# rsasaki0109/lidarslam_ros2

Measured on AMD Instinct MI355X. Metric: scan registrations/sec (30k-pt scan vs 10-frame submap), higher is better.
Workload: dtype f32; 1 GPU; cfg2: single NDT align(), 30000-pt VLP-32 scan (vg 0.2) vs 10-frame submap (vg 0.1), ndt_resolution 5.0, DIRECT7, max_iterations 30, transformation_epsilon 0; 1018 different scans (stream of 64); target_points=661519, voxels_valid=643, derivative_passes_last_scan=242, parallelism=1 registration stream per GPU x1, collective=none (one rank)

## Files before the change

lidarslam_ros2_amd/csrc/ndt.hip:

```cpp
#include "ndt.hpp"

#include <cmath>
#include <cstdlib>
#include <type_traits>

#include "grid_device.hpp"
#include "ndt_point.hpp"
#include "sort.hpp"

namespace lsr {

namespace {

__host__ __device__ inline void angle_tables(const double* p, bool with_hessian, int d1_sign, float* jang, float* hang) {
  double cx, cy, cz, sx, sy, sz;
  if (fabs(p[3]) < 10e-5) { cx = 1.0; sx = 0.0; } else { cx = cos(p[3]); sx = sin(p[3]); }
  if (fabs(p[4]) < 10e-5) { cy = 1.0; sy = 0.0; } else { cy = cos(p[4]); sy = sin(p[4]); }
  if (fabs(p[5]) < 10e-5) { cz = 1.0; sz = 0.0; } else { cz = cos(p[5]); sz = sin(p[5]); }
  jang[0] = (float)(-sx * sz + cx * sy * cz); jang[1] = (float)(-sx * cz - cx * sy * sz); jang[2] = (float)(-cx * cy);
  jang[3] = (float)(cx * sz + sx * sy * cz);  jang[4] = (float)(cx * cz - sx * sy * sz);  jang[5] = (float)(-sx * cy);
  jang[6] = (float)(-sy * cz);                jang[7] = (float)(sy * sz);                 jang[8] = (float)(cy);
  jang[9] = (float)(sx * cy * cz);            jang[10] = (float)(-sx * cy * sz);          jang[11] = (float)(sx * sy);
  jang[12] = (float)(-cx * cy * cz);          jang[13] = (float)(cx * cy * sz);           jang[14] = (float)(-cx * sy);
  jang[15] = (float)(-cy * sz);               jang[16] = (float)(-cy * cz);               jang[17] = 0.f;
// ... 413 lines not shown
  const double psi_t = phi_t - phi_0 - mu * d_phi_0 * a_t;
  const double d_psi_t = d_phi_t - mu * d_phi_0;
  if (phase == PH_MT_TRIAL || phase == PH_MT_LAST) {
    if (open_interval && (psi_t <= 0 && d_psi_t >= 0)) {
      open_interval = 0;
      I.f_l = I.f_l + phi_0 - mu * d_phi_0 * I.a_l;
      I.g_l = I.g_l + mu * d_phi_0;
      I.f_u = I.f_u + phi_0 - mu * d_phi_0 * I.a_u;
      I.g_u = I.g_u + mu * d_phi_0;
    }
    if (open_interval)
      interval_converged = mt_update_interval(I, a_t, psi_t, d_psi_t) ? 1 : 0;
    else
      interval_converged = mt_update_interval(I, a_t, phi_t, d_phi_t) ? 1 : 0;
    step_iterations++;
  }
  int next = CTL_DONE;
  if (!interval_converged && step_iterations < max_step_iterations && !(psi_t <= 0 && d_phi_t <= -nu * d_phi_0)) {
    if (open_interval)
      a_t = mt_trial_value(I.a_l, I.f_l, I.g_l, I.a_u, I.f_u, I.g_u, a_t, psi_t, d_psi_t);
    else
      a_t = mt_trial_value(I.a_l, I.f_l, I.g_l, I.a_u, I.f_u, I.g_u, a_t, phi_t, d_phi_t);
    a_t = fmax(fmin(a_t, step_max), step_min);
#pragma unroll
    for (int i = 0; i < 6; i++) S->x_t[i] = p[i] + dir[i] * a_t;
    S->a_t = a_t;
    const bool last = step_iterations + 1 >= max_step_iterations;
    S->want_hessian = last ? NDT_PASS_FUSED : NDT_PASS_GRAD;
    S->phase = last ? PH_MT_LAST : PH_MT_TRIAL;
    S->pad1 = 1;
  } else if (phase == PH_MT_LAST) {
    next = CTL_NEWTON_END;
  } else if (step_iterations) {
    S->want_hessian = 1;
    S->phase = PH_MT_HESS;
  } else {
    next = CTL_NEWTON_END;
  }
  S->n_evals = n_evals;
  S->n_passes = n_passes;
  S->last_pairs = sv[7];
  S->score = score;
#pragma unroll
  for (int i = 0; i < 6; i++) S->g[i] = sv[1 + i];
  S->open_interval = open_interval;
  S->interval_converged = interval_converged;
  S->step_iterations = step_iterations;
  S->a_l = I.a_l; S->f_l = I.f_l; S->g_l = I.g_l; S->a_u = I.a_u; S->f_u = I.f_u; S->g_u = I.g_u;
  return next;
}

__device__ __forceinline__ int ndt_newton_end(LdsState* S) {
  const int nr_iterations = S->nr_iterations, max_iter = S->max_iter;
  const double a_t = S->a_t, eps = S->eps;
  double p[6], dir[6];
#pragma unroll
  for (int i = 0; i < 6; i++) { p[i] = S->p[i]; dir[i] = S->dir[i]; }
  const double score = S->score;
  const int n_points = S->n_points;
  int converged = S->converged;
  if (nr_iterations > max_iter || (nr_iterations && (fabs(a_t) < eps))) converged = 1;
#pragma unroll
  for (int i = 0; i < 6; i++) S->p[i] = p[i] + dir[i] * a_t;
  S->nr_iterations = nr_iterations + 1;
  S->converged = converged;
  if (converged) {
    S->trans_probability = score / (double)n_points;
    S->done = 1;
    return CTL_DONE;
  }
  return CTL_NEWTON_BEGIN;
}

__device__ __forceinline__ int ndt_newton_begin(LdsState* S, const LdsDouble* delta_lds) {
  const double mu = 1.e-4;
  double delta[6], g[6], p[6];
#pragma unroll
  for (int i = 0; i < 6; i++) { delta[i] = delta_lds[i]; g[i] = S->g[i]; p[i] = S->p[i]; }
  const double score = S->score, step_max = S->step_max, step_min = S->step_min;
  const int n_points = S->n_points;
  double nrm = 0;
#pragma unroll
  for (int i = 0; i < 6; i++) nrm += delta[i] * delta[i];
  nrm = sqrt(nrm);
  if (nrm == 0 || nrm != nrm) {
    S->converged = (nrm == nrm) ? 1 : 0;
    S->trans_probability = score / (double)n_points;
    S->done = 1;
    return CTL_DONE;
  }
  double dir[6];
#pragma unroll
  for (int i = 0; i < 6; i++) dir[i] = delta[i] / nrm;
  const double phi_0 = -score;
  double dot = 0;
#pragma unroll
  for (int i = 0; i < 6; i++) dot += g[i] * dir[i];
  double d_phi_0 = -dot;
  S->phi_0 = phi_0;
  if (d_phi_0 >= 0) {
    if (d_phi_0 == 0) {
      S->d_phi_0 = d_phi_0;
      S->a_t = 0;
#pragma unroll
      for (int i = 0; i < 6; i++) S->dir[i] = dir[i];
      return CTL_NEWTON_END;
    }
    d_phi_0 = -d_phi_0;
#pragma unroll
    for (int i = 0; i < 6; i++) dir[i] = -dir[i];
  }
  const double a_t = fmax(fmin(nrm, step_max), step_min);
  S->d_phi_0 = d_phi_0;
  S->a_l = 0; S->a_u = 0;
  S->f_l = 0; S->f_u = 0;
  S->g_l = d_phi_0 - mu * d_phi_0;
  S->g_u = d_phi_0 - mu * d_phi_0;
  S->interval_converged = (step_max - step_min) < 0 ? 1 : 0;
  S->open_interval = 1;
  S->step_iterations = 0;
  S->a_t = a_t;
#pragma unroll
  for (int i = 0; i < 6; i++) { S->dir[i] = dir[i]; S->x_t[i] = p[i] + dir[i] * a_t; }
  S->want_hessian = 1;
  S->phase = PH_MT_FIRST;
  S->pad1 = 3;
  return CTL_DONE;
}

__device__ __forceinline__ void ndt_controller_wave0(LdsState* S, const LdsDouble* sums) {
  const bool lead = (threadIdx.x == 0);
  int next = 0;
  if (lead) next = ndt_controller_mt(S, sums);
  next = __builtin_amdgcn_readfirstlane(next);
  LdsDouble* scratch = const_cast<LdsDouble*>(sums);
  for (int guard = 0; guard < 8 && next != CTL_DONE; guard++) {
    if (next == CTL_NEWTON_END) {
      if (lead) next = ndt_newton_end(S);
    } else {
      asm volatile("s_waitcnt lgkmcnt(0)" ::: "memory");
      __builtin_amdgcn_wave_barrier();
      solve6_wave(sums + 8, S->g, scratch);
      asm volatile("s_waitcnt lgkmcnt(0)" ::: "memory");
      __builtin_amdgcn_wave_barrier();
      if (lead) next = ndt_newton_begin(S, scratch);
    }
    next = __builtin_amdgcn_readfirstlane(next);
  }
  if (lead && next != CTL_DONE) {
    S->trans_probability = S->score / (double)S->n_points;
    S->done = 1;
  }
}

#ifdef LSR_TIMING
__device__ long long* g_lsr_timing = nullptr;
#define LSR_STAMP(k)                                                                   \
  if (threadIdx.x == 0 && g_lsr_timing && blockIdx.y == 0) {                            \
    g_lsr_timing[blockIdx.x * 32 + 2 * (k)] = (long long)wall_clock64();                \
    g_lsr_timing[blockIdx.x * 32 + 2 * (k) + 1] = (long long)clock64();                 \
  }
#define LSR_STAMP_T(k, t)                                                              \
  if ((int)threadIdx.x == (t) && g_lsr_timing && blockIdx.y == 0) {                       \
    g_lsr_timing[blockIdx.x * 32 + 2 * (k)] = (long long)wall_clock64();                \
  }
#ifdef LSR_TIMING_SPAN
#define LSR_SPAN_BEGIN(seq)                                                                                   \
  if (threadIdx.x == 0 && g_lsr_timing && blockIdx.y == 0)                                                     \
    atomicMin((unsigned long long*)&g_lsr_timing[(512 + ((seq) & 255)) * 32 + 0], (unsigned long long)wall_clock64());
#define LSR_SPAN_END(seq)                                                                                     \
  if (threadIdx.x == 0 && g_lsr_timing && blockIdx.y == 0)                                                     \
    atomicMax((unsigned long long*)&g_lsr_timing[(512 + ((seq) & 255)) * 32 + 1], (unsigned long long)wall_clock64());
#else
#define LSR_SPAN_BEGIN(seq)
#define LSR_SPAN_END(seq)
#endif
#define LSR_CTL_BEGIN(L)                                                              \
  long long _ctl_t0 = 0; int _ctl_ph = 0;                                              \
  if (threadIdx.x == 0 && g_lsr_timing && blockIdx.x == 0 && blockIdx.y == 0) { _ctl_t0 = (long long)wall_clock64(); _ctl_ph = (L)->phase; }
#define LSR_CTL_END(col)                                                              \
  if (threadIdx.x == 0 && g_lsr_timing && blockIdx.x == 0 && blockIdx.y == 0) {          \
    const long long _t = (long long)wall_clock64();                                     \
    atomicAdd((unsigned long long*)&g_lsr_timing[(800 + _ctl_ph) * 32 + (col)], (unsigned long long)(_t - _ctl_t0)); \
    if ((col) == 0) atomicAdd((unsigned long long*)&g_lsr_timing[(800 + _ctl_ph) * 32 + 1], 1ull);                     \
    _ctl_t0 = _t;                                                                       \
  }
#define LSR_PASS_BEGIN()                                                               \
  long long _p_t0 = 0, _p_c0 = 0, _p_t1 = 0, _p_t7 = 0, _p_t2 = 0;                         \
  const bool _p_on = (threadIdx.x == 0 && g_lsr_timing && blockIdx.x == 0 && blockIdx.y == 0); \
  if (_p_on) { _p_t0 = (long long)wall_clock64(); _p_c0 = (long long)clock64(); }
#define LSR_PASS_MARK(var) if (_p_on) { var = (long long)wall_clock64(); }
#define LSR_PASS_END(hess)                                                             \
  if (_p_on) {                                                                          \
    const long long _t3 = (long long)wall_clock64(), _c3 = (long long)clock64();         \
    unsigned long long* _r = (unsigned long long*)&g_lsr_timing[(810 + ((hess) ? 1 : 0)) * 32]; \
    atomicAdd(&_r[0], 1ull); atomicAdd(&_r[1], (unsigned long long)(_p_t1 - _p_t0)); atomicAdd(&_r[2], (unsigned long long)(_p_t2 - _p_t7)); \
    atomicAdd(&_r[3], (unsigned long long)(_t3 - _p_t2)); atomicAdd(&_r[4], (unsigned long long)(_c3 - _p_c0)); atomicAdd(&_r[5], (unsigned long long)(_t3 - _p_t0)); \
  }
#else
#define LSR_STAMP(k)
#define LSR_STAMP_T(k, t)
#define LSR_SPAN_BEGIN(seq)
#define LSR_SPAN_END(seq)
#define LSR_CTL_BEGIN(L)
#define LSR_CTL_END(col)
#define LSR_PASS_BEGIN()
#define LSR_PASS_MARK(var)
#define LSR_PASS_END(hess)
#endif

__device__ __forceinline__ int uniform_i(int v) { return __builtin_amdgcn_readfirstlane(v); }
__device__ __forceinline__ float uniform_f(float v) { return __int_as_float(__builtin_amdgcn_readfirstlane(__float_as_int(v))); }
__device__ __forceinline__ double uniform_d(double v) {
  const int lo = __builtin_amdgcn_readfirstlane(__double2loint(v)), hi = __builtin_amdgcn_readfirstlane(__double2hiint(v));
  return __hiloint2double(hi, lo);
}

template <int CTRL>
__device__ __forceinline__ double dpp_quad_xor(double v) {
  int lo = __double2loint(v), hi = __double2hiint(v);
  lo = __builtin_amdgcn_update_dpp(0, lo, CTRL, 0xF, 0xF, true);
  hi = __builtin_amdgcn_update_dpp(0, hi, CTRL, 0xF, 0xF, true);
  return __hiloint2double(hi, lo);
}

template <int NOFF>
struct Offsets;
template <>
struct Offsets<1> {
  static __device__ __forceinline__ void get(int o, int& dx, int& dy, int& dz) { dx = dy = dz = 0; }
};
template <>
struct Offsets<7> {
  static __device__ __forceinline__ void get(int o, int& dx, int& dy, int& dz) {
    dx = (o == 1) - (o == 2);
    dy = (o == 3) - (o == 4);
    dz = (o == 5) - (o == 6);
  }
};
template <>
struct Offsets<27> {
  static __device__ __forceinline__ void get(int o, int& dx, int& dy, int& dz) {
    dx = o / 9 - 1;
    dy = (o / 3) % 3 - 1;
    dz = o % 3 - 1;
  }
};

namespace canon {
constexpr int TILE_PITCH = 68;
constexpr int TILE_ROWS = 16;
constexpr int TILE_FLOATS = TILE_ROWS * TILE_PITCH;

__device__ __forceinline__ double quantum(const int k) { return __hiloint2double((1023 + 62 - 31 * (k + 1)) << 20, 0); }
__device__ __forceinline__ double iquantum(const int k) { return __hiloint2double((1023 - 62 + 31 * (k + 1)) << 20, 0); }

__device__ __forceinline__ int piece(const double t, const int k, bool* poison) {
  *poison = !(fabs(t) < 4611686018427387904.0);
  if (*poison) return 0;
  double r = t;
  if (k > 0) r = t - trunc(t * iquantum(k - 1)) * quantum(k - 1);
  return (int)(r * iquantum(k));
}

__device__ __forceinline__ double reduce_grad(const float* p) {
  typedef float f4 __attribute__((ext_vector_type(4)));
  const f4 a = *reinterpret_cast<const f4*>(p), b = *reinterpret_cast<const f4*>(p + 4);
  double t = (double)a.x;
  t += (double)a.y; t += (double)a.z; t += (double)a.w;
  t += (double)b.x; t += (double)b.y; t += (double)b.z; t += (double)b.w;
  t += dpp_quad_xor<0xB1>(t);
  t += dpp_quad_xor<0x4E>(t);
  t += dpp_quad_xor<0x141>(t);
  return t;
}
__device__ __forceinline__ double reduce_hess(const float* p) {
  typedef float f4 __attribute__((ext_vector_type(4)));
  const f4 a = *reinterpret_cast<const f4*>(p), b = *reinterpret_cast<const f4*>(p + 4), c = *reinterpret_cast<const f4*>(p + 8),
           d = *reinterpret_cast<const f4*>(p + 12);
  double t = (double)a.x;
  t += (double)a.y; t += (double)a.z; t += (double)a.w;
  t += (double)b.x; t += (double)b.y; t += (double)b.z; t += (double)b.w;
  t += (double)c.x; t += (double)c.y; t += (double)c.z; t += (double)c.w;
  t += (double)d.x; t += (double)d.y; t += (double)d.z; t += (double)d.w;
  t += dpp_quad_xor<0xB1>(t);
  t += dpp_quad_xor<0x4E>(t);
  return t;
}
__device__ __forceinline__ void add_piece_lds(unsigned long long* ibin, const int v, const int k, const double t) {
  bool poison;
  const int m = piece(t, k, &poison);
  if (m != 0) atomicAdd(&ibin[k * 32 + v], (unsigned long long)(long long)m);
  if (poison && k == 0) atomicAdd(&ibin[31], 1ull);
}
}


__device__ __forceinline__ float dpp_quad_sum(float v) {
  v += __int_as_float(__builtin_amdgcn_update_dpp(0, __float_as_int(v), 0xB1, 0xF, 0xF, true));
  v += __int_as_float(__builtin_amdgcn_update_dpp(0, __float_as_int(v), 0x4E, 0xF, 0xF, true));
  return v;
}

template <int NOFF, int TAB, int PTS, bool KD = false>
__global__ __launch_bounds__(4 * PTS) void ndt_eval_quad_kernel(const NdtProblem P, const int seq) {
  constexpr int THREADS = 4 * PTS;
  constexpr int PITCH_PT = PTS + 8, PITCH_O = PTS + 4;
  constexpr int NT = (NOFF + 3) / 4;
  static_assert(PTS % 64 == 0, "a workgroup batch is a whole number of canonical chunks");
  if ((int)blockIdx.x >= P.nblocks) return;
  const int tid = threadIdx.x, ql = tid & 3, pq = tid >> 2;
  LSR_STAMP(0)
  LSR_STAMP_T(9, THREADS - 64)
  LSR_PASS_BEGIN()
  LSR_SPAN_BEGIN(seq)

  __shared__ float s_pt[14][PITCH_PT];
  __shared__ __attribute__((aligned(16))) float s_o[29][PITCH_O];
  __shared__ double s_bin[NDT_NBINS][32];
  __shared__ unsigned long long s_ibin[NDT_NBINS * 32];
  __shared__ double s_sum[NDT_NRED];
  __shared__ double s_lu[8][2];
  constexpr int STATE_Q = (int)(sizeof(NdtState) / 16);
  __shared__ uint4 s_state_q[STATE_Q];
  unsigned int* s_state = reinterpret_cast<unsigned int*>(s_state_q);
  extern __shared__ uint4 s_table[];

  const NdtState* __restrict__ Sin = P.st + (seq & 1);
  NdtState* __restrict__ Sout = P.st + ((seq + 1) & 1);

  const int stride = P.nblocks * PTS;
  int i = blockIdx.x * PTS + pq;
  float x = 0.f, y = 0.f, z = 0.f;
  unsigned int ang_entry = 0u, ang_entry_b = 0u;
  {
    const uint4* gq = reinterpret_cast<const uint4*>(Sin);
    const uint4 stq = (tid < STATE_Q) ? gq[tid] : make_uint4(0u, 0u, 0u, 0u);
    long long msum = 0;
    if (seq > 0 && tid < NDT_NBINS * 32) {
      const long long* b = P.bins + (size_t)((seq + 2) % NDT_NBANKS) * NDT_BANK_WORDS + tid;
      long long m[NDT_NSHARDS];
#pragma unroll
      for (int sh = 0; sh < NDT_NSHARDS; sh++) m[sh] = b[sh * (NDT_NBINS * 32)];
      msum = ((m[0] + m[1]) + (m[2] + m[3])) + ((m[4] + m[5]) + (m[6] + m[7]));
    }
    if (tid < NDT_NBINS * 32) {
      const int k = tid >> 5;
      const double q = __hiloint2double((1023 + 62 - 31 * (k + 1)) << 20, 0);
      s_bin[k][tid & 31] = (double)msum * q;
      s_ibin[tid] = 0ull;
    }
    if (tid < STATE_Q) s_state_q[tid] = stq;
    if (i < P.n) { x = P.sx[i]; y = P.sy[i]; z = P.sz[i]; }
    if (tid < 64) ang_entry = k_angle_entries[tid];
    if (tid < 8) ang_entry_b = k_angle_entries[64 + tid];
  }
  LSR_STAMP_T(8, 0)
  LSR_STAMP_T(10, THREADS - 64)
  barrier_lds_only();
  LdsState* L = (LdsState*)s_state;
  LSR_STAMP(1)
  LSR_PASS_MARK(_p_t1)
  if (P.mailbox != nullptr && blockIdx.x == 0 && tid == 0)
    __hip_atomic_store(&P.mailbox->progress, ((unsigned long long)(unsigned int)L->token << 32) | (unsigned int)seq,
                       __ATOMIC_RELAXED, __HIP_MEMORY_SCOPE_SYSTEM);
  if (uniform_i(L->done)) {
    if (blockIdx.x == 0 && seq > 0) {
      uint4* gq = reinterpret_cast<uint4*>(Sout);
      if (tid < STATE_Q) gq[tid] = s_state_q[tid];
    }
    return;
  }
  if (TAB == NDT_TAB_LDS) {
    const int nchunks = P.lds_bytes >> 10;
    const unsigned char* img = reinterpret_cast<const unsigned char*>(P.lds_image) + (size_t)(tid & 63) * 16;
    unsigned char* dst = reinterpret_cast<unsigned char*>(s_table);
    if (tid >= 64)
      for (int c = (tid >> 6) - 1; c < nchunks; c += THREADS / 64 - 1)
        __builtin_amdgcn_global_load_lds((const __attribute__((address_space(1))) void*)(img + (size_t)c * 1024),
                                         (__attribute__((address_space(3))) void*)(dst + (size_t)c * 1024), 16, 0, 0);
  }
  if (tid < 64) {
    if (seq > 0) {
      if (tid < NDT_NRED) {
        double t = (((s_bin[4][tid] + s_bin[3][tid]) + s_bin[2][tid]) + s_bin[1][tid]) + s_bin[0][tid];
        if (s_bin[0][31] != 0.0 || s_bin[1][31] != 0.0) t = __longlong_as_double(0x7FF8000000000000ll);
        s_sum[tid] = t;
      }
      wave_lds_fence();
      LSR_STAMP(6)
      LSR_CTL_BEGIN(L)
      ndt_controller_wave0(L, (const LdsDouble*)s_sum);
      wave_lds_fence();
      LSR_CTL_END(0)
      LSR_STAMP(5)
      build_request_wave0(reinterpret_cast<NdtState*>(s_state), &s_lu[0][0], reinterpret_cast<float*>(&s_lu[4][0]), ang_entry, ang_entry_b);
      LSR_CTL_END(2)
      LSR_STAMP(4)
    }
    if (blockIdx.x == 0) {
      uint4* gq = reinterpret_cast<uint4*>(Sout);
      gq[tid] = s_state_q[tid];
      if (tid + 64 < STATE_Q) gq[tid + 64] = s_state_q[tid + 64];
    }
  }
  __syncthreads();
  if (uniform_i(L->done)) {
    if (P.mailbox != nullptr && blockIdx.x == 0 && tid == 0) {
      NdtMailbox* mb = P.mailbox;
#pragma unroll
      for (int k = 0; k < 16; k++) mb->final_T[k] = L->final_T[k];
      mb->converged = L->converged;
      mb->nr_iterations = L->nr_iterations;
      mb->n_evals = L->n_evals;
      mb->n_passes = L->n_passes;
      mb->trans_probability = L->trans_probability;
      mb->last_pairs = L->last_pairs;
      __threadfence_system();
      __hip_atomic_store(&mb->done, (unsigned int)L->token, __ATOMIC_RELEASE, __HIP_MEMORY_SCOPE_SYSTEM);
    }
    return;
  }
  if (blockIdx.x == 0) {
    uint4* zb = reinterpret_cast<uint4*>(P.bins + (size_t)((seq + 1) % NDT_NBANKS) * NDT_BANK_WORDS);
    for (int k = tid; k < NDT_BANK_WORDS / 2; k += THREADS) zb[k] = make_uint4(0u, 0u, 0u, 0u);
  }
  LSR_STAMP(7)
  LSR_PASS_MARK(_p_t7)

  const int form = uniform_i(L->want_hessian);
  const bool hess = form != NDT_PASS_GRAD;
  const bool fused = form == NDT_PASS_FUSED;
  const double d1d = uniform_d(L->d1);
  const float d2 = uniform_f((float)L->d2);
  float T[12];
#pragma unroll
  for (int k = 0; k < 12; k++) T[k] = uniform_f(L->T[k]);
  const float leaf = P.leaf;
  LSR_STAMP(11)

  const unsigned short* s_map = reinterpret_cast<const unsigned short*>(s_table);
  const float4* s_rec = reinterpret_cast<const float4*>(reinterpret_cast<const unsigned char*>(s_table) + P.lds_map_bytes);

  long long* const bank = P.bins + (size_t)(seq % NDT_NBANKS) * NDT_BANK_WORDS + (size_t)(blockIdx.x & (NDT_NSHARDS - 1)) * (NDT_NBINS * 32);
  const bool one_batch = (long long)blockIdx.x * PTS + stride >= (long long)P.n;
  for (int base = blockIdx.x * PTS; base < P.n; base += stride) {
    {
      const float tx = xform_ref(T[0], T[1], T[2], T[3], x, y, z);
      const float ty = xform_ref(T[4], T[5], T[6], T[7], x, y, z);
      const float tz = xform_ref(T[8], T[9], T[10], T[11], x, y, z);
      const float fx = floorf(tx / leaf), fy = floorf(ty / leaf), fz = floorf(tz / leaf);
      const bool finite_ok = (i < P.n) && (fabsf(fx) < 1.0e9f) && (fabsf(fy) < 1.0e9f) && (fabsf(fz) < 1.0e9f);
      const int ci = finite_ok ? (int)fx : INT_MIN / 2, cj = finite_ok ? (int)fy : INT_MIN / 2, ck = finite_ok ? (int)fz : INT_MIN / 2;

      bool valid[NT], score_only[NT];
      int cellv[NT];
#pragma unroll
      for (int t = 0; t < NT; t++) {
        score_only[t] = false;
        const int o = ql + 4 * t;
        int dx, dy, dz;
        Offsets<NOFF>::get(o, dx, dy, dz);
        const int a = ci + dx, b = cj + dy, c = ck + dz;
        const bool in = (o < NOFF) & (a >= P.min_b[0]) & (a <= P.max_b[0]) & (b >= P.min_b[1]) & (b <= P.max_b[1]) &
                        (c >= P.min_b[2]) & (c <= P.max_b[2]);
        valid[t] = in;
        cellv[t] = in ? ((a - P.min_b[0]) + (b - P.min_b[1]) * P.mul1 + (c - P.min_b[2]) * P.mul2) : 0;
      }
      if (KD) {
#pragma unroll
        for (int t = 0; t < NT; t++) {
          const int code = valid[t] ? P.cell_slot[cellv[t]] : -1, sl = kd_slot(code);
          const float4 cen = P.centroid[sl >= 0 ? sl : 0];
          valid[t] = (sl >= 0) & centroid_in_radius(tx, ty, tz, cen.x, cen.y, cen.z, P.radius2);
          score_only[t] = valid[t] & (code < -1);
        }
      }
      float4 r0[NT], r1[NT], r2[NT];
      if (TAB == NDT_TAB_LDS) {
        int slot[NT];
#pragma unroll
        for (int t = 0; t < NT; t++) {
          const int sl = (int)s_map[cellv[t]];
          valid[t] = valid[t] & (sl != 0xFFFF);
          slot[t] = valid[t] ? sl : 0;
        }
#pragma unroll
        for (int t = 0; t < NT; t++) {
          r0[t] = s_rec[slot[t] * 3 + 0];
          r1[t] = s_rec[slot[t] * 3 + 1];
          r2[t] = s_rec[slot[t] * 3 + 2];
        }
      } else {
        size_t ridx[NT];
#pragma unroll
        for (int t = 0; t < NT; t++) {
          if (TAB != NDT_TAB_COMPACT) {
            ridx[t] = (size_t)cellv[t];
          } else {
            const int sl = P.cell_slot[cellv[t]];
            valid[t] = valid[t] & (sl >= 0);
            ridx[t] = (size_t)(sl >= 0 ? sl : 0);
          }
        }
#pragma unroll
        for (int t = 0; t < NT; t++) {
          r0[t] = P.rec[ridx[t] * 4 + 0];
          r1[t] = P.rec[ridx[t] * 4 + 1];
          r2[t] = P.rec[ridx[t] * 4 + 2];
        }
      }

      if (KD) {
#pragma unroll
        for (int t = 0; t < NT; t++) {
          if (score_only[t]) {
            valid[t] = true;
            r0[t] = r1[t] = r2[t] = make_float4(0.f, 0.f, 0.f, 0.f);
          }
        }
      }
      float score = 0.f, npairs = 0.f;
      float A0 = 0.f, A1 = 0.f, A2 = 0.f;
      float E00 = 0.f, E01 = 0.f, E02 = 0.f, E11 = 0.f, E12 = 0.f, E22 = 0.f;
#pragma unroll
      for (int t = 0; t < NT; t++)
        pair_terms(valid[t], hess, tx, ty, tz, r0[t], r1[t], r2[t], d2, d1d, score, npairs, A0, A1, A2, E00, E01, E02, E11, E12, E22);
      score = dpp_quad_sum(score); npairs = dpp_quad_sum(npairs);
      A0 = dpp_quad_sum(A0); A1 = dpp_quad_sum(A1); A2 = dpp_quad_sum(A2);
      if (hess) {
        E00 = dpp_quad_sum(E00); E01 = dpp_quad_sum(E01); E02 = dpp_quad_sum(E02);
        E11 = dpp_quad_sum(E11); E12 = dpp_quad_sum(E12); E22 = dpp_quad_sum(E22);
        const float row0 = (ql == 0) ? score : (ql == 1) ? npairs : (ql == 2) ? A0 : A1;
        const float row1 = (ql == 0) ? A2 : (ql == 1) ? E00 : (ql == 2) ? E01 : E02;
        const float row2 = (ql == 0) ? E11 : (ql == 1) ? E12 : (ql == 2) ? E22 : x;
        s_pt[ql][pq] = row0;
        s_pt[4 + ql][pq] = row1;
        s_pt[8 + ql][pq] = row2;
        if (ql < 2) s_pt[12 + ql][pq] = (ql == 0) ? y : z;
      } else {
        float o[29];
        if (npairs != 0.f) {
          point_terms(false, x, y, z, score, npairs, A0, A1, A2, 0.f, 0.f, 0.f, 0.f, 0.f, 0.f, L->jang, L->hang, o);
        } else {
#pragma unroll
          for (int k = 0; k < NDT_NRED_GRAD; k++) o[k] = 0.f;
        }
        s_o[ql][pq] = (ql == 0) ? o[0] : (ql == 1) ? o[1] : (ql == 2) ? o[2] : o[3];
        s_o[4 + ql][pq] = (ql == 0) ? o[4] : (ql == 1) ? o[5] : (ql == 2) ? o[6] : o[7];
      }
      i += stride;
      x = 0.f; y = 0.f; z = 0.f;
      if (i < P.n) { x = P.sx[i]; y = P.sy[i]; z = P.sz[i]; }
    }
    LSR_STAMP(12)
    barrier_lds_only();
    if (hess) {
      if (tid < PTS) {
        const float npairs = s_pt[1][tid];
        float o[29];
        if (npairs != 0.f) {
          point_terms(true, s_pt[11][tid], s_pt[12][tid], s_pt[13][tid], s_pt[0][tid], npairs, s_pt[2][tid], s_pt[3][tid], s_pt[4][tid],
                      s_pt[5][tid], s_pt[6][tid], s_pt[7][tid], s_pt[8][tid], s_pt[9][tid], s_pt[10][tid], L->jang, L->hang, o);
        } else {
#pragma unroll
          for (int k = 0; k < 29; k++) o[k] = 0.f;
        }
#pragma unroll
        for (int k = 0; k < 29; k++) s_o[k][tid] = o[k];
      }
      LSR_STAMP(13)
      barrier_lds_only();
    }
    LSR_STAMP(14)
    if (!hess || fused) {
      constexpr int RUNS = PTS / 8;
      if (tid < NDT_NRED_GRAD * RUNS) {
        const int v = tid / RUNS, k = tid & 7;
        const double t = canon::reduce_grad(&s_o[v][8 * (tid % RUNS)]);
        bool poison;
        long long m = canon::piece(t, k < NDT_NBINS ? k : 0, &poison);
        int pz = poison ? 1 : 0;
        if (PTS == 128) { m += (long long)__shfl_xor((int)m, 8, 64); pz |= __shfl_xor(pz, 8, 64); }
        if ((tid & (RUNS - 1)) < NDT_NBINS) {
          unsigned long long* dst = one_batch ? reinterpret_cast<unsigned long long*>(bank) : s_ibin;
          if (m != 0) atomicAdd(dst + k * 32 + v, (unsigned long long)m);
          if (pz && k == 0) atomicAdd(dst + 31, 1ull);
        }
      }
    }
    if (hess) {
      constexpr int RUNS = PTS / 16;
      static_assert(NDT_NRED_GRAD * (PTS / 8) % 64 == 0 && NDT_NRED_GRAD * (PTS / 8) + (((29 - NDT_NRED_GRAD) * RUNS + 63) & ~63) <= THREADS,
                    "fused pass: the two trees sit on whole waves of their own");
      const int v0 = fused ? NDT_NRED_GRAD : 0;
      const int ht = tid - (fused ? NDT_NRED_GRAD * (PTS / 8) : 0);
      if (ht >= 0 && ht < (((29 - v0) * RUNS + 63) & ~63)) {
        const int v = v0 + ht / RUNS, sg = tid & 3;
        double t = 0.0;
        if (v < 29) t = canon::reduce_hess(&s_o[v][16 * (tid % RUNS)]);
        bool poison, poison0;
        long long m = canon::piece(t, sg + 1, &poison);
        long long m0 = canon::piece(t, 0, &poison0);
        int pz = poison0 ? 1 : 0;
        if (PTS == 128) {
          m += (long long)__shfl_xor((int)m, 4, 64); m0 += (long long)__shfl_xor((int)m0, 4, 64); pz |= __shfl_xor(pz, 4, 64);
        }
        if (v < 29 && (tid & (RUNS - 1)) < 4) {
          unsigned long long* dst = one_batch ? reinterpret_cast<unsigned long long*>(bank) : s_ibin;
          if (m != 0) atomicAdd(dst + (sg + 1) * 32 + v, (unsigned long long)m);
          if (sg == 0) {
            if (m0 != 0) atomicAdd(dst + v, (unsigned long long)m0);
            if (pz) atomicAdd(dst + 31, 1ull);
          }
        }
      }
    }
    if (!hess && base + stride < P.n) barrier_lds_only();
  }

  LSR_STAMP(2)
  LSR_PASS_MARK(_p_t2)
  if (!one_batch) {
    __syncthreads();
    if (tid < NDT_NBINS * 32) {
      const unsigned long long m = s_ibin[tid];
      if (m != 0ull) atomicAdd(reinterpret_cast<unsigned long long*>(bank + tid), m);
    }
  }
  LSR_STAMP(3)
  LSR_PASS_END(hess)
  LSR_SPAN_END(seq)
}

typedef float v4f __attribute__((ext_vector_type(4)));
typedef __attribute__((address_space(3))) const v4f LdsV4;
typedef __attribute__((address_space(1))) const v4f GlbV4;
typedef __attribute__((address_space(1))) const float GlbFloat;
typedef __attribute__((address_space(1))) const int GlbInt;

template <int NOFF, int TAB, int THREADS, bool BYVAL, bool SPLIT = false, bool KD = false>
__global__ __launch_bounds__(THREADS) __attribute__((amdgpu_waves_per_eu(4))) void ndt_eval_lane_kernel(const NdtProblem pv, const NdtProblem* __restrict__ probs, const int seq,
                                                                const int nb, const int tab_bytes) {
  constexpr int NWAVES = THREADS / 64;
  constexpr int PTS = SPLIT ? THREADS / 2 : THREADS;
  constexpr int NT = (NOFF + 3) / 4;
  constexpr int GROUP = 4;
  const NdtProblem& P = BYVAL ? pv : probs[blockIdx.y];
  const int tid = threadIdx.x, lane = tid & 63, wave = tid >> 6;
  if (blockIdx.x > 0 && (long long)blockIdx.x * PTS >= (long long)P.n) return;
  const int role = SPLIT ? (wave & 1) : 0;
  const int cw = SPLIT ? (wave >> 1) : wave;

  __shared__ double s_bin[NDT_NBINS][32];
  __shared__ unsigned long long s_ibin[NDT_NBINS * 32];
  __shared__ double s_sum[NDT_NRED];
  __shared__ double s_lu[8][2];
  constexpr int STATE_Q = (int)(sizeof(NdtState) / 16);
  static_assert(STATE_Q <= THREADS, "NdtState copy assumes <= THREADS uint4");
  __shared__ uint4 s_state_q[STATE_Q];
  unsigned int* s_state = reinterpret_cast<unsigned int*>(s_state_q);
  extern __shared__ uint4 s_table[];

  const NdtState* __restrict__ Sin = P.st + (seq & 1);
  NdtState* __restrict__ Sout = P.st + ((seq + 1) & 1);

  const int n = P.n;
  const int stride = nb * PTS;
  int i = blockIdx.x * PTS + cw * 64 + lane;
  float x = 0.f, y = 0.f, z = 0.f;
  unsigned int ang_entry = 0u, ang_entry_b = 0u;
  {
    const uint4* gq = reinterpret_cast<const uint4*>(Sin);
    const uint4 stq = (tid < STATE_Q) ? gq[tid] : make_uint4(0u, 0u, 0u, 0u);
    long long msum = 0;
    if (seq > 0 && tid < NDT_NBINS * 32) {
      const long long* b = P.bins + (size_t)((seq + 2) % NDT_NBANKS) * NDT_BANK_WORDS + tid;
      long long m[NDT_NSHARDS];
#pragma unroll
      for (int sh = 0; sh < NDT_NSHARDS; sh++) m[sh] = b[sh * (NDT_NBINS * 32)];
      msum = ((m[0] + m[1]) + (m[2] + m[3])) + ((m[4] + m[5]) + (m[6] + m[7]));
    }
    if (tid < NDT_NBINS * 32) {
      s_bin[tid >> 5][tid & 31] = (double)msum * canon::quantum(tid >> 5);
      s_ibin[tid] = 0ull;
    }
    if (tid < STATE_Q) s_state_q[tid] = stq;
    if (i < n) { x = P.sx[i]; y = P.sy[i]; z = P.sz[i]; }
    if (tid < 64) ang_entry = k_angle_entries[tid];
    if (tid < 8) ang_entry_b = k_angle_entries[64 + tid];
  }
  barrier_lds_only();
  LdsState* L = (LdsState*)s_state;
  if (P.mailbox != nullptr && blockIdx.x == 0 && tid == 0)
    __hip_atomic_store(&P.mailbox->progress, ((unsigned long long)(unsigned int)L->token << 32) | (unsigned int)seq,
                       __ATOMIC_RELAXED, __HIP_MEMORY_SCOPE_SYSTEM);
  if (uniform_i(L->done)) {
    if (blockIdx.x == 0 && seq > 0) {
      uint4* gq = reinterpret_cast<uint4*>(Sout);
      if (tid < STATE_Q) gq[tid] = s_state_q[tid];
    }
    return;
  }
  if (TAB == NDT_TAB_LDS) {
    const int nchunks = P.lds_bytes >> 10;
    const unsigned char* img = reinterpret_cast<const unsigned char*>(P.lds_image) + (size_t)lane * 16;
    unsigned char* dst = reinterpret_cast<unsigned char*>(s_table);
    if (tid >= 64)
      for (int c = wave - 1; c < nchunks; c += NWAVES - 1)
        __builtin_amdgcn_global_load_lds((const __attribute__((address_space(1))) void*)(img + (size_t)c * 1024),
                                         (__attribute__((address_space(3))) void*)(dst + (size_t)c * 1024), 16, 0, 0);
  }
  if (tid < 64) {
    if (seq > 0) {
      if (tid < NDT_NRED) {
        double t = (((s_bin[4][tid] + s_bin[3][tid]) + s_bin[2][tid]) + s_bin[1][tid]) + s_bin[0][tid];
        if (s_bin[0][31] != 0.0 || s_bin[1][31] != 0.0) t = __longlong_as_double(0x7FF8000000000000ll);
        s_sum[tid] = t;
      }
      wave_lds_fence();
      ndt_controller_wave0(L, (const LdsDouble*)s_sum);
      wave_lds_fence();
      build_request_wave0(reinterpret_cast<NdtState*>(s_state), &s_lu[0][0], reinterpret_cast<float*>(&s_lu[4][0]), ang_entry, ang_entry_b);
    }
    if (blockIdx.x == 0) {
      uint4* gq = reinterpret_cast<uint4*>(Sout);
      gq[tid] = s_state_q[tid];
      if (tid + 64 < STATE_Q) gq[tid + 64] = s_state_q[tid + 64];
    }
  }
  __syncthreads();
  if (uniform_i(L->done)) {
    if (P.mailbox != nullptr && blockIdx.x == 0 && tid == 0) {
      NdtMailbox* mb = P.mailbox;
#pragma unroll
      for (int k = 0; k < 16; k++) mb->final_T[k] = L->final_T[k];
      mb->converged = L->converged;
      mb->nr_iterations = L->nr_iterations;
      mb->n_evals = L->n_evals;
      mb->n_passes = L->n_passes;
      mb->trans_probability = L->trans_probability;
      mb->last_pairs = L->last_pairs;
      __threadfence_system();
      __hip_atomic_store(&mb->done, (unsigned int)L->token, __ATOMIC_RELEASE, __HIP_MEMORY_SCOPE_SYSTEM);
    }
    return;
  }
  if (blockIdx.x == 0) {
    uint4* zb = reinterpret_cast<uint4*>(P.bins + (size_t)((seq + 1) % NDT_NBANKS) * NDT_BANK_WORDS);
    for (int k = tid; k < NDT_BANK_WORDS / 2; k += THREADS) zb[k] = make_uint4(0u, 0u, 0u, 0u);
  }

  const int form = uniform_i(L->want_hessian);
  const bool hess = form != NDT_PASS_GRAD;
  const bool fused = form == NDT_PASS_FUSED;
  const double d1d = uniform_d(L->d1);
  const float d2 = uniform_f((float)L->d2);
  float T[12];
#pragma unroll
  for (int k = 0; k < 12; k++) T[k] = uniform_f(L->T[k]);
  const float leaf = P.leaf;
  const int mb0 = P.min_b[0], mb1 = P.min_b[1], mb2 = P.min_b[2];
  const int xb0 = P.max_b[0], xb1 = P.max_b[1], xb2 = P.max_b[2];
  const int mul1 = P.mul1, mul2 = P.mul2;
  const __attribute__((address_space(3))) unsigned short* s_map = (const __attribute__((address_space(3))) unsigned short*)s_table;
  const int map_bytes = P.lds_map_bytes;
  float* s_tile = reinterpret_cast<float*>(reinterpret_cast<unsigned char*>(s_table) + tab_bytes) + wave * canon::TILE_FLOATS;
  const GlbV4* g_rec = (const GlbV4*)P.rec;
  const GlbInt* g_cell_slot = (const GlbInt*)P.cell_slot;
  const GlbFloat* g_sx = (const GlbFloat*)P.sx;
  const GlbFloat* g_sy = (const GlbFloat*)P.sy;
  const GlbFloat* g_sz = (const GlbFloat*)P.sz;
  (void)g_rec; (void)g_cell_slot; (void)s_map; (void)map_bytes;

  for (int base = SPLIT ? blockIdx.x * PTS : blockIdx.x * PTS + cw * 64; base < n; base += stride) {
    const bool have = i < n;
    const float px = x, py = y, pz = z;
    const float tx = xform_ref(T[0], T[1], T[2], T[3], px, py, pz);
    const float ty = xform_ref(T[4], T[5], T[6], T[7], px, py, pz);
    const float tz = xform_ref(T[8], T[9], T[10], T[11], px, py, pz);
    i += stride;
    if (i < n) { x = g_sx[i]; y = g_sy[i]; z = g_sz[i]; }
    const float fx = floorf(tx / leaf), fy = floorf(ty / leaf), fz = floorf(tz / leaf);
    const bool finite_ok = have && (fabsf(fx) < 1.0e9f) && (fabsf(fy) < 1.0e9f) && (fabsf(fz) < 1.0e9f);
    const int ci = finite_ok ? (int)fx : INT_MIN / 2, cj = finite_ok ? (int)fy : INT_MIN / 2, ck = finite_ok ? (int)fz : INT_MIN / 2;
    bool inx[3], iny[3], inz[3];
#pragma unroll
    for (int d = 0; d < 3; d++) {
      inx[d] = (ci + d - 1 >= mb0) & (ci + d - 1 <= xb0);
      iny[d] = (cj + d - 1 >= mb1) & (cj + d - 1 <= xb1);
      inz[d] = (ck + d - 1 >= mb2) & (ck + d - 1 <= xb2);
    }
    const int centre = (ci - mb0) + (cj - mb1) * mul1 + (ck - mb2) * mul2;

    bool nb_ok[NOFF], nb_so[NOFF];
    int nb_rec[NOFF];
#pragma unroll
    for (int o = 0; o < NOFF; o++) {
      int dx, dy, dz;
      Offsets<NOFF>::get(o, dx, dy, dz);
      const bool in = inx[dx + 1] & iny[dy + 1] & inz[dz + 1];
      const int cell = in ? centre + dx + dy * mul1 + dz * mul2 : 0;
      nb_ok[o] = in;
      nb_so[o] = false;
      nb_rec[o] = cell;
    }
    if (KD) {
#pragma unroll
      for (int o = 0; o < NOFF; o++) {
        const int code = nb_ok[o] ? P.cell_slot[nb_rec[o]] : -1, ks = kd_slot(code);
        const float4 cen = P.centroid[ks >= 0 ? ks : 0];
        nb_ok[o] = (ks >= 0) & centroid_in_radius(tx, ty, tz, cen.x, cen.y, cen.z, P.radius2);
        nb_so[o] = nb_ok[o] & (code < -1);
      }
    }
    if (TAB == NDT_TAB_LDS) {
      int sl[NOFF];
#pragma unroll
      for (int o = 0; o < NOFF; o++) sl[o] = (int)s_map[nb_rec[o]];
#pragma unroll
      for (int o = 0; o < NOFF; o++) {
        nb_ok[o] = nb_ok[o] & (sl[o] != 0xFFFF);
        nb_rec[o] = map_bytes + (nb_ok[o] ? sl[o] : 0) * NDT_LDS_REC_BYTES;
      }
    } else if (TAB == NDT_TAB_COMPACT) {
      int sl[NOFF];
#pragma unroll
      for (int o = 0; o < NOFF; o++) sl[o] = g_cell_slot[nb_rec[o]];
#pragma unroll
      for (int o = 0; o < NOFF; o++) {
        nb_ok[o] = nb_ok[o] & (sl[o] >= 0);
        nb_rec[o] = sl[o] >= 0 ? sl[o] : 0;
      }
    }

    if (KD) {
#pragma unroll
      for (int o = 0; o < NOFF; o++) nb_ok[o] = nb_ok[o] | nb_so[o];
    }

    bool nb_any[NOFF];
#pragma unroll
    for (int o = 0; o < NOFF; o++) nb_any[o] = __builtin_amdgcn_ballot_w64(nb_ok[o]) != 0ull;

    float S[11];
#pragma unroll
    for (int half = 0; half < 2; half++) {
      if (SPLIT && half != role) continue;
      float Pq[2][11];
#pragma unroll
      for (int k = 0; k < 11; k++) { Pq[0][k] = 0.f; Pq[1][k] = 0.f; }
#pragma unroll
      for (int e0 = 0; e0 < 2 * NT; e0 += GROUP) {
        v4f r0[GROUP], r1[GROUP], r2[GROUP];
#pragma unroll
        for (int u = 0; u < GROUP; u++) {
          const int e = e0 + u, ql = e / NT, t = e % NT, o = 2 * half + ql + 4 * t;
          if (e < 2 * NT && o < NOFF) {
            if (TAB == NDT_TAB_LDS) {
              const LdsV4* rp = (const LdsV4*)((const __attribute__((address_space(3))) unsigned char*)s_table + nb_rec[o]);
              r0[u] = rp[0]; r1[u] = rp[1]; r2[u] = rp[2];
            } else {
              const GlbV4* rp = g_rec + (size_t)nb_rec[o] * 4;
              r0[u] = rp[0]; r1[u] = rp[1]; r2[u] = rp[2];
            }
            if (KD && nb_so[o]) {
              const v4f z = {0.f, 0.f, 0.f, 0.f};
              r0[u] = z; r1[u] = z; r2[u] = z;
            }
          }
        }
#pragma unroll
        for (int u = 0; u < GROUP; u++) {
          const int e = e0 + u, ql = e / NT, t = e % NT, o = 2 * half + ql + 4 * t;
          if (e < 2 * NT && o < NOFF && nb_any[o]) {
            float* A = Pq[ql];
            pair_terms(nb_ok[o], hess, tx, ty, tz, make_float4(r0[u].x, r0[u].y, r0[u].z, r0[u].w), make_float4(r1[u].x, r1[u].y, r1[u].z, r1[u].w),
                       make_float4(r2[u].x, r2[u].y, r2[u].z, r2[u].w), d2, d1d, A[0], A[1], A[2], A[3], A[4], A[5], A[6], A[7], A[8], A[9], A[10]);
          }
        }
      }
      if (half == 0 || SPLIT) {
#pragma unroll
        for (int k = 0; k < 11; k++) S[k] = Pq[0][k] + Pq[1][k];
      } else {
#pragma unroll
        for (int k = 0; k < 11; k++) S[k] = S[k] + (Pq[0][k] + Pq[1][k]);
      }
    }
    if (SPLIT) {
      if (role == 1) {
#pragma unroll
        for (int k = 0; k < 11; k++) s_tile[k * canon::TILE_PITCH + lane] = S[k];
      }
      __syncthreads();
      if (role == 1) {
        if (base + stride < n) __syncthreads();
        continue;
      }
      const float* other = s_tile + canon::TILE_FLOATS;
#pragma unroll
      for (int k = 0; k < 11; k++) S[k] = S[k] + other[k * canon::TILE_PITCH + lane];
      if (base + stride < n) __syncthreads();
    }
    float o[29];
    {
      const bool any_pair = S[1] != 0.f;
      const float qx = any_pair ? px : 0.f, qy = any_pair ? py : 0.f, qz = any_pair ? pz : 0.f;
      point_terms(hess, qx, qy, qz, S[0], S[1], S[2], S[3], S[4], S[5], S[6], S[7], S[8], S[9], S[10], L->jang, L->hang, o);
    }
    if (!hess) {
#pragma unroll
      for (int k = 0; k < NDT_NRED_GRAD; k++) s_tile[k * canon::TILE_PITCH + lane] = o[k];
      wave_lds_fence();
      const int v = lane >> 3, g = lane & 7;
      const double t = canon::reduce_grad(s_tile + v * canon::TILE_PITCH + 8 * g);
// ... 224 lines not shown
```

Measured before the change: 455.9 registrations/s.

## Precompute per-lane LDS addresses and reduction constants in kernel prologue, pin with asm holds

Moves per-lane address and index work out of the per-pass loop and into the kernel prologue, computed while the head waves' bin loads are in flight: LDS addresses, neighbour-offset cell deltas, reduction-tree source/destination offsets and quantisation constants. Empty asm constraints keep these values in VGPRs/SGPRs and force kernel arguments into scalar registers. Cell indices become a base index plus a precomputed delta, and shfl_xor is replaced with ds_swizzle. This trades extra live registers, which could lower occupancy, for fewer integer ops and address calculations on the hot path.

```diff
diff --git a/lidarslam_ros2_amd/csrc/ndt.hip b/lidarslam_ros2_amd/csrc/ndt.hip
--- a/lidarslam_ros2_amd/csrc/ndt.hip
+++ b/lidarslam_ros2_amd/csrc/ndt.hip
@@ -739,12 +739,40 @@
   return v;
 }
 
+__device__ __forceinline__ void hold(int& v) { asm volatile("" : "+v"(v)); }
+__device__ __forceinline__ void hold(unsigned int& v) { asm volatile("" : "+v"(v)); }
+__device__ __forceinline__ void hold(double& v) { asm volatile("" : "+v"(v)); }
+__device__ __forceinline__ void hold_uniform(int& v) { asm volatile("" : "+s"(v)); }
+__device__ __forceinline__ void hold_uniform(unsigned int& v) { asm volatile("" : "+s"(v)); }
+typedef __attribute__((address_space(3))) float LdsFloat;
+__device__ __forceinline__ unsigned int lds_addr(const void* p) {
+  return (unsigned int)(unsigned long long)(__attribute__((address_space(3))) const void*)p;
+}
+__device__ __forceinline__ LdsFloat* lds_float(unsigned int a) { return (LdsFloat*)(unsigned long long)a; }
+__device__ __forceinline__ int piece_held(const double t, const bool rest, const double iq_prev, const double q_prev, const double iq,
+                                          bool* poison) {
+  *poison = !(fabs(t) < 4611686018427387904.0);
+  if (*poison) return 0;
+  double r = t;
+  if (rest) r = t - trunc(t * iq_prev) * q_prev;
+  return (int)(r * iq);
+}
+template <int X>
+__device__ __forceinline__ int swizzle_xor(int v) { return __builtin_amdgcn_ds_swizzle(v, (X << 10) | 0x1f); }
+
 template <int NOFF, int TAB, int PTS, bool KD = false>
 __global__ __launch_bounds__(4 * PTS) void ndt_eval_quad_kernel(const NdtProblem P, const int seq) {
   constexpr int THREADS = 4 * PTS;
   constexpr int PITCH_PT = PTS + 8, PITCH_O = PTS + 4;
   constexpr int NT = (NOFF + 3) / 4;
   static_assert(PTS % 64 == 0, "a workgroup batch is a whole number of canonical chunks");
+  asm volatile("" ::"s"(P.sx), "s"(P.sy), "s"(P.sz), "s"(P.n), "s"(P.nblocks), "s"(P.min_b[0]), "s"(P.min_b[1]), "s"(P.min_b[2]),
+               "s"(P.max_b[0]), "s"(P.max_b[1]), "s"(P.max_b[2]), "s"(P.mul1), "s"(P.mul2), "s"(P.leaf), "s"(P.bins), "s"(P.st),
+               "s"(P.mailbox), "s"(seq));
+  if (TAB == NDT_TAB_LDS) asm volatile("" ::"s"(P.lds_image), "s"(P.lds_bytes), "s"(P.lds_map_bytes));
+  if (TAB != NDT_TAB_LDS) asm volatile("" ::"s"(P.rec));
+  if (TAB == NDT_TAB_COMPACT || KD) asm volatile("" ::"s"(P.cell_slot));
+  if (KD) asm volatile("" ::"s"(P.centroid), "s"(P.radius2));
   if ((int)blockIdx.x >= P.nblocks) return;
   const int tid = threadIdx.x, ql = tid & 3, pq = tid >> 2;
   LSR_STAMP(0)
@@ -765,22 +793,70 @@
 
   const NdtState* __restrict__ Sin = P.st + (seq & 1);
   NdtState* __restrict__ Sout = P.st + ((seq + 1) & 1);
-
   const int stride = P.nblocks * PTS;
   int i = blockIdx.x * PTS + pq;
+
+  unsigned int a_pt, a_o, b_pt, b_o;
+  int ndx[NT], ndy[NT], ndz[NT];
+  unsigned int ndelta[NT];
+  constexpr int RUNS_G = PTS / 8, RUNS_H = PTS / 16;
+  int g_k, g_send;
+  unsigned int g_src, g_dst;
+  double g_iq, g_iqp, g_qp;
+  constexpr int H_LANE0 = NDT_NRED_GRAD * (PTS / 8), H_VSHIFT = NDT_NRED_GRAD - H_LANE0 / RUNS_H;
+  static_assert(H_LANE0 % RUNS_H == 0, "fused pass: the Hessian tree starts on a run boundary");
+  int h_v, h_send;
+  unsigned int h_src, h_dst, h_dst0;
+  double h_iq, h_iqp, h_qp;
+  unsigned int bank_w = (unsigned int)(seq % NDT_NBANKS) * NDT_BANK_WORDS + (blockIdx.x & (NDT_NSHARDS - 1)) * (NDT_NBINS * 32);
+  unsigned int clear_w = (unsigned int)((seq + 1) % NDT_NBANKS) * NDT_BANK_WORDS;
+  int one_batch_i = uniform_i(((long long)blockIdx.x * PTS + stride >= (long long)P.n) ? 1 : 0);
+  hold_uniform(bank_w); hold_uniform(clear_w); hold_uniform(one_batch_i);
+  auto lane_constants = [&]() __attribute__((always_inline)) {
+    a_pt = lds_addr(&s_pt[ql][pq]); a_o = lds_addr(&s_o[ql][pq]);
+    b_pt = lds_addr(&s_pt[0][0]) + 4u * (unsigned int)tid; b_o = lds_addr(&s_o[0][0]) + 4u * (unsigned int)tid;
+    hold(a_pt); hold(a_o); hold(b_pt); hold(b_o);
+#pragma unroll
+    for (int t = 0; t < NT; t++) {
+      Offsets<NOFF>::get(ql + 4 * t, ndx[t], ndy[t], ndz[t]);
+      ndelta[t] = (unsigned int)ndx[t] + (unsigned int)ndy[t] * (unsigned int)P.mul1 + (unsigned int)ndz[t] * (unsigned int)P.mul2;
+      if (NOFF > 1) { hold(ndx[t]); hold(ndy[t]); hold(ndz[t]); hold(ndelta[t]); }
+    }
+    const int gv = tid / RUNS_G;
+    g_k = (tid & 7) < NDT_NBINS ? (tid & 7) : 0;
+    g_src = lds_addr(&s_o[0][0]) + 4u * (unsigned int)(gv * PITCH_O + 8 * (tid % RUNS_G));
+    g_dst = 8u * (unsigned int)((tid & 7) * 32 + gv);
+    g_send = ((tid & (RUNS_G - 1)) < NDT_NBINS) ? 1 : 0;
+    g_iq = canon::iquantum(g_k); g_iqp = canon::iquantum(g_k > 0 ? g_k - 1 : 0); g_qp = canon::quantum(g_k > 0 ? g_k - 1 : 0);
+    hold(g_k); hold(g_src); hold(g_dst); hold(g_send); hold(g_iq); hold(g_iqp); hold(g_qp);
+    const int sg = tid & 3;
+    h_v = tid / RUNS_H;
+    h_src = lds_addr(&s_o[0][0]) + 4u * (unsigned int)(h_v * PITCH_O + 16 * (tid % RUNS_H));
+    h_dst = 8u * (unsigned int)((sg + 1) * 32 + h_v); h_dst0 = 8u * (unsigned int)h_v;
+    h_send = ((tid & (RUNS_H - 1)) < 4) ? 1 + sg : 0;
+    h_iq = canon::iquantum(sg + 1); h_iqp = canon::iquantum(sg); h_qp = canon::quantum(sg);
+    hold(h_v); hold(h_src); hold(h_dst); hold(h_dst0); hold(h_send); hold(h_iq); hold(h_iqp); hold(h_qp);
+  };
+
+  constexpr int HEAD_WAVES = 3;
+  static_assert(NDT_NBINS * 32 <= HEAD_WAVES * 64 && STATE_Q <= HEAD_WAVES * 64, "the waves behind the head waves carry no head loads");
+  const int wave = uniform_i(tid >> 6);
   float x = 0.f, y = 0.f, z = 0.f;
   unsigned int ang_entry = 0u, ang_entry_b = 0u;
-  {
+  if (wave < HEAD_WAVES) {
     const uint4* gq = reinterpret_cast<const uint4*>(Sin);
     const uint4 stq = (tid < STATE_Q) ? gq[tid] : make_uint4(0u, 0u, 0u, 0u);
-    long long msum = 0;
+    long long m[NDT_NSHARDS];
+#pragma unroll
+    for (int sh = 0; sh < NDT_NSHARDS; sh++) m[sh] = 0;
     if (seq > 0 && tid < NDT_NBINS * 32) {
       const long long* b = P.bins + (size_t)((seq + 2) % NDT_NBANKS) * NDT_BANK_WORDS + tid;
-      long long m[NDT_NSHARDS];
 #pragma unroll
       for (int sh = 0; sh < NDT_NSHARDS; sh++) m[sh] = b[sh * (NDT_NBINS * 32)];
-      msum = ((m[0] + m[1]) + (m[2] + m[3])) + ((m[4] + m[5]) + (m[6] + m[7]));
-    }
+    }
+    asm volatile("" ::: "memory");
+    lane_constants();
+    const long long msum = ((m[0] + m[1]) + (m[2] + m[3])) + ((m[4] + m[5]) + (m[6] + m[7]));
     if (tid < NDT_NBINS * 32) {
       const int k = tid >> 5;
       const double q = __hiloint2double((1023 + 62 - 31 * (k + 1)) << 20, 0);
@@ -788,10 +864,12 @@
       s_ibin[tid] = 0ull;
     }
     if (tid < STATE_Q) s_state_q[tid] = stq;
-    if (i < P.n) { x = P.sx[i]; y = P.sy[i]; z = P.sz[i]; }
-    if (tid < 64) ang_entry = k_angle_entries[tid];
-    if (tid < 8) ang_entry_b = k_angle_entries[64 + tid];
-  }
+  } else {
+    lane_constants();
+  }
+  if (i < P.n) { x = P.sx[i]; y = P.sy[i]; z = P.sz[i]; }
+  if (tid < 64) ang_entry = k_angle_entries[tid];
+  if (tid < 8) ang_entry_b = k_angle_entries[64 + tid];
   LSR_STAMP_T(8, 0)
   LSR_STAMP_T(10, THREADS - 64)
   barrier_lds_only();
@@ -859,7 +937,7 @@
     return;
   }
   if (blockIdx.x == 0) {
-    uint4* zb = reinterpret_cast<uint4*>(P.bins + (size_t)((seq + 1) % NDT_NBANKS) * NDT_BANK_WORDS);
+    uint4* zb = reinterpret_cast<uint4*>(P.bins + clear_w);
     for (int k = tid; k < NDT_BANK_WORDS / 2; k += THREADS) zb[k] = make_uint4(0u, 0u, 0u, 0u);
   }
   LSR_STAMP(7)
@@ -879,8 +957,10 @@
   const unsigned short* s_map = reinterpret_cast<const unsigned short*>(s_table);
   const float4* s_rec = reinterpret_cast<const float4*>(reinterpret_cast<const unsigned char*>(s_table) + P.lds_map_bytes);
 
-  long long* const bank = P.bins + (size_t)(seq % NDT_NBANKS) * NDT_BANK_WORDS + (size_t)(blockIdx.x & (NDT_NSHARDS - 1)) * (NDT_NBINS * 32);
-  const bool one_batch = (long long)blockIdx.x * PTS + stride >= (long long)P.n;
+  long long* const bank = P.bins + bank_w;
+  const bool one_batch = one_batch_i != 0;
+  char* const bank_b = reinterpret_cast<char*>(bank);
+  char* const ibin_b = reinterpret_cast<char*>(s_ibin);
   for (int base = blockIdx.x * PTS; base < P.n; base += stride) {
     {
       const float tx = xform_ref(T[0], T[1], T[2], T[3], x, y, z);
@@ -892,17 +972,17 @@
 
       bool valid[NT], score_only[NT];
       int cellv[NT];
+      const unsigned int cell0 = ((unsigned int)ci - (unsigned int)P.min_b[0]) + ((unsigned int)cj - (unsigned int)P.min_b[1]) * (unsigned int)P.mul1 +
+                                 ((unsigned int)ck - (unsigned int)P.min_b[2]) * (unsigned int)P.mul2;
 #pragma unroll
       for (int t = 0; t < NT; t++) {
         score_only[t] = false;
         const int o = ql + 4 * t;
-        int dx, dy, dz;
-        Offsets<NOFF>::get(o, dx, dy, dz);
-        const int a = ci + dx, b = cj + dy, c = ck + dz;
+        const int a = ci + ndx[t], b = cj + ndy[t], c = ck + ndz[t];
         const bool in = (o < NOFF) & (a >= P.min_b[0]) & (a <= P.max_b[0]) & (b >= P.min_b[1]) & (b <= P.max_b[1]) &
                         (c >= P.min_b[2]) & (c <= P.max_b[2]);
         valid[t] = in;
-        cellv[t] = in ? ((a - P.min_b[0]) + (b - P.min_b[1]) * P.mul1 + (c - P.min_b[2]) * P.mul2) : 0;
+        cellv[t] = in ? (int)(cell0 + ndelta[t]) : 0;
       }
       if (KD) {
 #pragma unroll
@@ -971,10 +1051,11 @@
         const float row0 = (ql == 0) ? score : (ql == 1) ? npairs : (ql == 2) ? A0 : A1;
         const float row1 = (ql == 0) ? A2 : (ql == 1) ? E00 : (ql == 2) ? E01 : E02;
         const float row2 = (ql == 0) ? E11 : (ql == 1) ? E12 : (ql == 2) ? E22 : x;
-        s_pt[ql][pq] = row0;
-        s_pt[4 + ql][pq] = row1;
-        s_pt[8 + ql][pq] = row2;
-        if (ql < 2) s_pt[12 + ql][pq] = (ql == 0) ? y : z;
+        LdsFloat* const w = lds_float(a_pt);
+        w[0] = row0;
+        w[4 * PITCH_PT] = row1;
+        w[8 * PITCH_PT] = row2;
+        if (ql < 2) w[12 * PITCH_PT] = (ql == 0) ? y : z;
       } else {
         float o[29];
         if (npairs != 0.f) {
@@ -983,8 +1064,9 @@
 #pragma unroll
           for (int k = 0; k < NDT_NRED_GRAD; k++) o[k] = 0.f;
         }
-        s_o[ql][pq] = (ql == 0) ? o[0] : (ql == 1) ? o[1] : (ql == 2) ? o[2] : o[3];
-        s_o[4 + ql][pq] = (ql == 0) ? o[4] : (ql == 1) ? o[5] : (ql == 2) ? o[6] : o[7];
+        LdsFloat* const w = lds_float(a_o);
+        w[0] = (ql == 0) ? o[0] : (ql == 1) ? o[1] : (ql == 2) ? o[2] : o[3];
+        w[4 * PITCH_O] = (ql == 0) ? o[4] : (ql == 1) ? o[5] : (ql == 2) ? o[6] : o[7];
       }
       i += stride;
       x = 0.f; y = 0.f; z = 0.f;
@@ -994,17 +1076,19 @@
     barrier_lds_only();
     if (hess) {
       if (tid < PTS) {
-        const float npairs = s_pt[1][tid];
+        const LdsFloat* const r = lds_float(b_pt);
+        LdsFloat* const w = lds_float(b_o);
+        const float npairs = r[1 * PITCH_PT];
         float o[29];
         if (npairs != 0.f) {
-          point_terms(true, s_pt[11][tid], s_pt[12][tid], s_pt[13][tid], s_pt[0][tid], npairs, s_pt[2][tid], s_pt[3][tid], s_pt[4][tid],
-                      s_pt[5][tid], s_pt[6][tid], s_pt[7][tid], s_pt[8][tid], s_pt[9][tid], s_pt[10][tid], L->jang, L->hang, o);
+          point_terms(true, r[11 * PITCH_PT], r[12 * PITCH_PT], r[13 * PITCH_PT], r[0], npairs, r[2 * PITCH_PT], r[3 * PITCH_PT], r[4 * PITCH_PT],
+                      r[5 * PITCH_PT], r[6 * PITCH_PT], r[7 * PITCH_PT], r[8 * PITCH_PT], r[9 * PITCH_PT], r[10 * PITCH_PT], L->jang, L->hang, o);
         } else {
 #pragma unroll
           for (int k = 0; k < 29; k++) o[k] = 0.f;
         }
 #pragma unroll
-        for (int k = 0; k < 29; k++) s_o[k][tid] = o[k];
+        for (int k = 0; k < 29; k++) w[k * PITCH_O] = o[k];
       }
       LSR_STAMP(13)
       barrier_lds_only();
@@ -1013,16 +1097,20 @@
     if (!hess || fused) {
       constexpr int RUNS = PTS / 8;
       if (tid < NDT_NRED_GRAD * RUNS) {
-        const int v = tid / RUNS, k = tid & 7;
-        const double t = canon::reduce_grad(&s_o[v][8 * (tid % RUNS)]);
+        const double t = canon::reduce_grad((const float*)lds_float(g_src));
         bool poison;
-        long long m = canon::piece(t, k < NDT_NBINS ? k : 0, &poison);
+        long long m = piece_held(t, g_k > 0, g_iqp, g_qp, g_iq, &poison);
         int pz = poison ? 1 : 0;
-        if (PTS == 128) { m += (long long)__shfl_xor((int)m, 8, 64); pz |= __shfl_xor(pz, 8, 64); }
-        if ((tid & (RUNS - 1)) < NDT_NBINS) {
-          unsigned long long* dst = one_batch ? reinterpret_cast<unsigned long long*>(bank) : s_ibin;
-          if (m != 0) atomicAdd(dst + k * 32 + v, (unsigned long long)m);
-          if (pz && k == 0) atomicAdd(dst + 31, 1ull);
+        if (PTS == 128) { m += (long long)swizzle_xor<8>((int)m); pz |= swizzle_xor<8>(pz); }
+        if (g_send) {
+          const bool first = g_k == 0;
+          if (one_batch) {
+            if (m != 0) atomicAdd(reinterpret_cast<unsigned long long*>(bank_b + g_dst), (unsigned long long)m);
+            if (pz && first) atomicAdd(reinterpret_cast<unsigned long long*>(bank_b + 31 * 8), 1ull);
+          } else {
+            if (m != 0) atomicAdd(reinterpret_cast<unsigned long long*>(ibin_b + g_dst), (unsigned long long)m);
+            if (pz && first) atomicAdd(reinterpret_cast<unsigned long long*>(ibin_b + 31 * 8), 1ull);
+          }
         }
       }
     }
@@ -1031,24 +1119,34 @@
       static_assert(NDT_NRED_GRAD * (PTS / 8) % 64 == 0 && NDT_NRED_GRAD * (PTS / 8) + (((29 - NDT_NRED_GRAD) * RUNS + 63) & ~63) <= THREADS,
                     "fused pass: the two trees sit on whole waves of their own");
       const int v0 = fused ? NDT_NRED_GRAD : 0;
-      const int ht = tid - (fused ? NDT_NRED_GRAD * (PTS / 8) : 0);
+      const int ht = tid - (fused ? H_LANE0 : 0);
       if (ht >= 0 && ht < (((29 - v0) * RUNS + 63) & ~63)) {
-        const int v = v0 + ht / RUNS, sg = tid & 3;
+        const int vs = fused ? H_VSHIFT : 0;
+        const int v = h_v + vs;
         double t = 0.0;
-        if (v < 29) t = canon::reduce_hess(&s_o[v][16 * (tid % RUNS)]);
+        if (v < 29) t = canon::reduce_hess((const float*)lds_float(h_src + (unsigned int)(vs * PITCH_O * 4)));
         bool poison, poison0;
-        long long m = canon::piece(t, sg + 1, &poison);
+        long long m = piece_held(t, true, h_iqp, h_qp, h_iq, &poison);
         long long m0 = canon::piece(t, 0, &poison0);
         int pz = poison0 ? 1 : 0;
         if (PTS == 128) {
-          m += (long long)__shfl_xor((int)m, 4, 64); m0 += (long long)__shfl_xor((int)m0, 4, 64); pz |= __shfl_xor(pz, 4, 64);
+          m += (long long)swizzle_xor<4>((int)m); m0 += (long long)swizzle_xor<4>((int)m0); pz |= swizzle_xor<4>(pz);
         }
-        if (v < 29 && (tid & (RUNS - 1)) < 4) {
-          unsigned long long* dst = one_batch ? reinterpret_cast<unsigned long long*>(bank) : s_ibin;
-          if (m != 0) atomicAdd(dst + (sg + 1) * 32 + v, (unsigned long long)m);
-          if (sg == 0) {
-            if (m0 != 0) atomicAdd(dst + v, (unsigned long long)m0);
-            if (pz) atomicAdd(dst + 31, 1ull);
+        if (v < 29 && h_send) {
+          const bool first = h_send == 1;
+          const unsigned int d = h_dst + (unsigned int)(vs * 8), d0 = h_dst0 + (unsigned int)(vs * 8);
+          if (one_batch) {
+            if (m != 0) atomicAdd(reinterpret_cast<unsigned long long*>(bank_b + d), (unsigned long long)m);
+            if (first) {
+              if (m0 != 0) atomicAdd(reinterpret_cast<unsigned long long*>(bank_b + d0), (unsigned long long)m0);
+              if (pz) atomicAdd(reinterpret_cast<unsigned long long*>(bank_b + 31 * 8), 1ull);
+            }
+          } else {
+            if (m != 0) atomicAdd(reinterpret_cast<unsigned long long*>(ibin_b + d), (unsigned long long)m);
+            if (first) {
+              if (m0 != 0) atomicAdd(reinterpret_cast<unsigned long long*>(ibin_b + d0), (unsigned long long)m0);
+              if (pz) atomicAdd(reinterpret_cast<unsigned long long*>(ibin_b + 31 * 8), 1ull);
+            }
           }
         }
       }
```

New measurement: 472.9 registrations/s (median of 6 runs). +3.7%, better.
